# krullgit/3D-Object-Detection-for-autonomous-navigation

Measured on AMD Instinct MI355X. Metric: frames/sec (whole node) + p50 per-frame ms, 16k-pt pillars, higher is better.
Workload: dtype f32 (GEMMs on the 16-bit matrix pipe as split operands -- two float16 pieces per value, 3 products, fp32 accumulate: fp32-equivalent results, measured 1.5e-6 max from the fp32 oracle at this shape)

## Files before the change

### 3d-object-detection-for-autonomous-navigation_amd/csrc/voxelize.hip

```cpp
#include "pp_common.h"

#define VT 1024
#define VWAVES 16
#define VL_PPT 16
#define VL_CAP (VT * VL_PPT)

__device__ __forceinline__ unsigned long long lanemask_lt() {
    unsigned lane = threadIdx.x & 63u;
    return (lane == 0) ? 0ull : (~0ull >> (64u - lane));
}

__global__ __launch_bounds__(256) void k_cell_first(const float* __restrict__ pts,
                                                    const int* __restrict__ offsets, int F, VoxGeom g,
                                                    int* __restrict__ cell, int* __restrict__ first,
                                                    int* __restrict__ cellmap, const PpFeed* __restrict__ feed,
                                                    float* __restrict__ pts_dst, int* __restrict__ offsets_dst,
                                                    unsigned long long* __restrict__ occbits, int occ_n) {
    const int b = blockIdx.y;
    if (feed != nullptr) {
        offsets = feed->offsets;
        pts = feed->src;
    }
    if (cellmap != nullptr) {
        int* cm = cellmap + (size_t)b * g.ncell;
        if ((g.ncell & 3) == 0) {
            const int4 m1 = make_int4(-1, -1, -1, -1);
            for (int e = blockIdx.x * 256 + threadIdx.x; e < (g.ncell >> 2); e += gridDim.x * 256) reinterpret_cast<int4*>(cm)[e] = m1;
        } else {
            for (int e = blockIdx.x * 256 + threadIdx.x; e < g.ncell; e += gridDim.x * 256) cm[e] = -1;
        }
    }
    if (occbits != nullptr)
        for (int e = blockIdx.x * 256 + threadIdx.x; e < occ_n; e += gridDim.x * 256) occbits[(size_t)b * occ_n + e] = 0ull;
    const int n0 = offsets[b];
    const int n1 = offsets[b + 1];
    const int n = n1 - n0;
    if (feed != nullptr && blockIdx.x == 0 && threadIdx.x == 0) {
        offsets_dst[b] = n0;
        if (b == (int)gridDim.y - 1) offsets_dst[b + 1] = n1;
    }
    const int i = blockIdx.x * 256 + threadIdx.x;
    if (i >= n) return;
    const float* ps_ = pts + (size_t)(n0 + i) * F;
    float p[3] = {ps_[0], ps_[1], ps_[2]};
    if (feed != nullptr) {
        float* q = pts_dst + (size_t)(n0 + i) * F;
        q[0] = p[0]; q[1] = p[1]; q[2] = p[2];
        for (int j = 3; j < F; ++j) q[j] = ps_[j];
    }
    int c3[3];
    bool ok = true;
#pragma unroll
    for (int j = 0; j < 3; ++j) {
        double c = floor(((double)p[j] - g.lo[j]) / g.vs[j]);
        if (!(c >= 0.0 && c < (double)g.grid[j])) ok = false;
        c3[j] = ok ? (int)c : 0;
    }
    int lin = -1;
    if (ok) {
        lin = (c3[2] * g.grid[1] + c3[1]) * g.grid[0] + c3[0];
        if (first != nullptr) atomicMin(&first[(size_t)b * g.ncell + lin], i);
    }
    cell[n0 + i] = lin;
}

__device__ __forceinline__ int block_excl_scan(int v, int* s_tmp, int& total) {
    const int lane = threadIdx.x & 63, wave = threadIdx.x >> 6;
    const int x = wave_inclusive_scan(v);
    if (lane == 63) s_tmp[wave] = x;
    __syncthreads();
    int woff = 0, tot = 0;
#pragma unroll
    for (int w = 0; w < VWAVES; ++w) {
        int t = s_tmp[w];
        if (w < wave) woff += t;
        tot += t;
    }
    __syncthreads();
    total = tot;
    return woff + x - v;
}

int voxel_sort_passes(int max_voxels) {
    int bits = 1;
    while ((1 << bits) < max_voxels) ++bits;
    return (bits + 7) / 8;
}

template <int BITS, int PPT>
__global__ __launch_bounds__(VT) void k_voxel_frame(
    const int* __restrict__ offsets, const int* __restrict__ cell, const int* __restrict__ first,
    int* __restrict__ cellmap, unsigned* keyA, unsigned* idxA, unsigned* keyB, unsigned* idxB,
    int* __restrict__ pillar_start, int* __restrict__ pillar_cell, int* __restrict__ npillars,
    int* __restrict__ nvalid_out, int ncell, int max_voxels, int npass, int bits_rt) {
    const int bits = (BITS > 0) ? BITS : bits_rt;
    __shared__ int s_tot[VWAVES];
    __shared__ int s_carry;
    __shared__ int s_break;
    __shared__ int s_tmp[VWAVES];
    __shared__ int s_hist[256 * VWAVES];
    constexpr int CAP = VT * PPT;
    constexpr bool TABLES = (PPT == 16);
    __shared__ unsigned s_sort[2 * VL_CAP];

    const int b = blockIdx.x;
    const int tid = threadIdx.x, lane = tid & 63, wave = tid >> 6;
    const int n0 = offsets[b];
    const int n = offsets[b + 1] - n0;
    const int* fcell = cell + n0;
    const int* ffirst = (first != nullptr) ? first + (size_t)b * ncell : nullptr;
    int* fmap = cellmap + (size_t)b * ncell;
    unsigned* kA = keyA + n0;
    unsigned* vA = idxA + n0;
    unsigned* kB = keyB + n0;
    unsigned* vB = idxB + n0;
    const unsigned long long lt = lanemask_lt();

    if (tid == 0) { s_carry = 0; s_break = 0x7fffffff; }
    __syncthreads();

    int ib = 1;
    while ((1 << ib) < n) ++ib;
    if (n <= CAP && npass * bits + ib <= 32 && (first != nullptr || (TABLES && ncell <= VL_CAP))) {
        const int ppt = (n + VT - 1) / VT;
        const int i0 = tid * ppt;
        int c[PPT];
        if (ppt == PPT && ((n0 | n) & 3) == 0 && i0 + PPT <= n) {
#pragma unroll
            for (int k = 0; k < PPT; k += 4) {
                const int4 v = *reinterpret_cast<const int4*>(fcell + i0 + k);
                c[k] = v.x; c[k + 1] = v.y; c[k + 2] = v.z; c[k + 3] = v.w;
            }
        } else {
#pragma unroll
            for (int k = 0; k < PPT; ++k) c[k] = (k < ppt && i0 + k < n) ? fcell[i0 + k] : -1;
        }
        int f[PPT];
        if (first != nullptr) {
#pragma unroll
            for (int k = 0; k < PPT; ++k) f[k] = (c[k] >= 0) ? ffirst[c[k]] : -1;
        } else {
            int* s_first = reinterpret_cast<int*>(s_sort) + VL_CAP;
            for (int e = tid; e < ncell; e += VT) s_first[e] = 0x7fffffff;
            __syncthreads();
#pragma unroll
            for (int k = 0; k < PPT; ++k) if (c[k] >= 0) atomicMin(&s_first[c[k]], i0 + k);
            __syncthreads();
#pragma unroll
            for (int k = 0; k < PPT; ++k) f[k] = (c[k] >= 0) ? s_first[c[k]] : -1;
            __syncthreads();
        }
        int* const s_map = reinterpret_cast<int*>(s_sort) + VL_CAP;
        unsigned flags = 0;
#pragma unroll
        for (int k = 0; k < PPT; ++k) if (c[k] >= 0 && f[k] == i0 + k) flags |= 1u << k;
        int totp;
        const int basep = block_excl_scan(__popc(flags), s_tmp, totp);
        {
            int r = 0;
#pragma unroll
            for (int k = 0; k < PPT; ++k)
                if ((flags >> k) & 1u) {
                    const int pid = basep + r++;
                    if (pid < max_voxels) {
                        fmap[c[k]] = pid;
                        if (first == nullptr) s_map[c[k]] = pid;
                        pillar_cell[(size_t)b * max_voxels + pid] = c[k];
                    } else if (pid == max_voxels) {
                        s_break = i0 + k;
                    }
                }
        }
        __syncthreads();
        const int P = min(totp, max_voxels);
        const int ibreak = s_break;
        unsigned vmask = 0;
#pragma unroll
        for (int k = 0; k < PPT; ++k) if (c[k] >= 0 && i0 + k < ibreak) vmask |= 1u << k;
        int key[PPT];
#pragma unroll
        for (int k = 0; k < PPT; ++k) key[k] = ((vmask >> k) & 1u) ? (first == nullptr ? s_map[c[k]] : fmap[c[k]]) : 0;
        int nv;
        const int basev = block_excl_scan(__popc(vmask), s_tmp, nv);
        {
            int r = 0;
#pragma unroll
            for (int k = 0; k < PPT; ++k)
                if ((vmask >> k) & 1u) s_sort[basev + r++] = ((unsigned)key[k] << ib) | (unsigned)(i0 + k);
        }
        __syncthreads();
        unsigned* const sk = s_sort;
        unsigned* const dk = s_sort;
        const int NB = 1 << bits;
        const unsigned dmask = (unsigned)NB - 1u;
        const int chunk = ((nv + VWAVES * 64 - 1) / (VWAVES * 64)) * 64;
        const int wbeg = min(wave * chunk, nv), wend = min(wbeg + chunk, nv);
        for (int pass = 0; pass < npass; ++pass) {
            const int shift = ib + pass * bits;
            for (int e = tid; e < NB * VWAVES; e += VT) s_hist[e] = 0;
            unsigned ev[PPT];
#pragma unroll
            for (int t = 0; t < PPT; ++t) {
                const int j = wbeg + t * 64 + lane;
                ev[t] = (j < wend) ? sk[j] : 0u;
            }
            __syncthreads();
            int rank[PPT], rbase[PPT];
            const unsigned lt_lo = (unsigned)lt, lt_hi = (unsigned)(lt >> 32);
#pragma unroll
            for (int t = 0; t < PPT; ++t) {
                rank[t] = 0;
                rbase[t] = 0;
                if (wbeg + t * 64 < wend) {
                    const bool act = wbeg + t * 64 + lane < wend;
                    const unsigned d = (ev[t] >> shift) & dmask;
                    const unsigned long long am = __builtin_amdgcn_ballot_w64(act);
                    unsigned plo = (unsigned)am, phi = (unsigned)(am >> 32);
                    if (BITS > 0) {
#pragma unroll
                        for (int bit = 0; bit < BITS; ++bit) {
                            const unsigned m = (unsigned)__builtin_amdgcn_sbfe((int)d, bit, 1);
                            const unsigned long long bb = __builtin_amdgcn_ballot_w64(__builtin_amdgcn_ubfe(d, bit, 1) != 0u);
                            plo &= ~((unsigned)bb ^ m);
                            phi &= ~((unsigned)(bb >> 32) ^ m);
                        }
                    } else {
                        for (int bit = 0; bit < bits; ++bit) {
                            const unsigned m = (unsigned)__builtin_amdgcn_sbfe((int)d, bit, 1);
                            const unsigned long long bb = __builtin_amdgcn_ballot_w64(__builtin_amdgcn_ubfe(d, bit, 1) != 0u);
                            plo &= ~((unsigned)bb ^ m);
                            phi &= ~((unsigned)(bb >> 32) ^ m);
                        }
                    }
                    if (act) {
                        int* hp = &s_hist[wave * NB + d];
                        rbase[t] = __hip_atomic_load(hp, __ATOMIC_RELAXED, __HIP_MEMORY_SCOPE_WORKGROUP);
                        const unsigned blo = plo & lt_lo, bhi = phi & lt_hi;
                        rank[t] = __popc(blo) + __popc(bhi);
                        if ((blo | bhi) == 0u)
                            __hip_atomic_fetch_add(hp, __popc(plo) + __popc(phi), __ATOMIC_RELAXED, __HIP_MEMORY_SCOPE_WORKGROUP);
                    }
                }
            }
#pragma unroll
            for (int t = 0; t < PPT; ++t) rank[t] += rbase[t];
            __syncthreads();
            {
                const int E = NB * VWAVES;
                const int per = (E + VT - 1) / VT;
                const int e0 = tid * per;
                int local = 0;
                for (int q = 0; q < per; ++q)
                    if (e0 + q < E) local += s_hist[((e0 + q) % VWAVES) * NB + (e0 + q) / VWAVES];
                int total;
                int run = block_excl_scan(local, s_tmp, total);
                for (int q = 0; q < per; ++q)
                    if (e0 + q < E) {
                        int* hp = &s_hist[((e0 + q) % VWAVES) * NB + (e0 + q) / VWAVES];
                        const int t = *hp;
                        *hp = run;
                        run += t;
                    }
            }
            __syncthreads();
#pragma unroll
            for (int t = 0; t < PPT; ++t) {
                if (wbeg + t * 64 + lane < wend) {
                    const unsigned d = (ev[t] >> shift) & dmask;
                    dk[s_hist[wave * NB + d] + rank[t]] = ev[t];
                }
            }
            __syncthreads();
        }
        int* ps = pillar_start + (size_t)b * (max_voxels + 1);
        const unsigned imask = (1u << ib) - 1u;
        unsigned* fin = ((npass & 1) ? idxB : idxA) + n0;
#pragma unroll
        for (int t = 0; t < PPT; ++t) {
            const int j = tid + t * VT;
            if (j < nv) {
                const unsigned v = sk[j];
                fin[j] = v & imask;
                const unsigned k = v >> ib;
                if (j == 0 || (sk[j - 1] >> ib) != k) ps[k] = j;
            }
        }
        if (tid == 0) {
            ps[P] = nv;
            npillars[b] = P;
            nvalid_out[b] = nv;
        }
        return;
    }

    for (int base = 0; base < n; base += VT) {
        const int i = base + tid;
        const int c = (i < n) ? fcell[i] : -1;
        const bool flag = (c >= 0) && (ffirst[c] == i);
        const unsigned long long bal = __ballot(flag);
        if (lane == 0) s_tot[wave] = __popcll(bal);
        __syncthreads();
        int woff = 0, tile_tot = 0;
#pragma unroll
        for (int w = 0; w < VWAVES; ++w) {
            int t = s_tot[w];
            if (w < wave) woff += t;
            tile_tot += t;
        }
        const int pid = s_carry + woff + __popcll(bal & lt);
        if (flag) {
            if (pid < max_voxels) {
                fmap[c] = pid;
                pillar_cell[(size_t)b * max_voxels + pid] = c;
            } else if (pid == max_voxels) {
                s_break = i;
            }
        }
        __syncthreads();
        if (tid == 0) s_carry += tile_tot;
    }
    __syncthreads();
    const int P = min(s_carry, max_voxels);
    const int ibreak = s_break;
    __syncthreads();

    if (tid == 0) s_carry = 0;
    __syncthreads();
    for (int base = 0; base < n; base += VT) {
        const int i = base + tid;
        const int c = (i < n) ? fcell[i] : -1;
        const bool valid = (c >= 0) && (i < ibreak);
        const unsigned long long bal = __ballot(valid);
        if (lane == 0) s_tot[wave] = __popcll(bal);
        __syncthreads();
        int woff = 0, tile_tot = 0;
#pragma unroll
        for (int w = 0; w < VWAVES; ++w) {
            int t = s_tot[w];
            if (w < wave) woff += t;
            tile_tot += t;
        }
        if (valid) {
            const int pos = s_carry + woff + __popcll(bal & lt);
            kA[pos] = (unsigned)fmap[c];
            vA[pos] = (unsigned)i;
        }
        __syncthreads();
        if (tid == 0) s_carry += tile_tot;
    }
    __syncthreads();
    const int nv = s_carry;
    __syncthreads();

    unsigned* sk = kA; unsigned* sv = vA; unsigned* dk = kB; unsigned* dv = vB;
    const int NB = 1 << bits;
    const unsigned dmask = (unsigned)NB - 1u;
    const int chunk = ((nv + VWAVES * 64 - 1) / (VWAVES * 64)) * 64;
    const int wbeg = min(wave * chunk, nv);
    const int wend = min(wbeg + chunk, nv);
    volatile int* vhist = s_hist;
    for (int pass = 0; pass < npass; ++pass) {
        const int shift = pass * bits;
        for (int e = tid; e < NB * VWAVES; e += VT) s_hist[e] = 0;
        __syncthreads();
        for (int t0 = wbeg; t0 < wend; t0 += 64) {
            const int j = t0 + lane;
            if (j < wend) atomicAdd(&s_hist[wave * NB + ((sk[j] >> shift) & dmask)], 1);
        }
        __syncthreads();
        {
            const int E = NB * VWAVES;
            const int per = (E + VT - 1) / VT;
            const int e0 = tid * per;
            int local = 0;
            for (int q = 0; q < per; ++q)
                if (e0 + q < E) local += s_hist[((e0 + q) % VWAVES) * NB + (e0 + q) / VWAVES];
            int total;
            int run = block_excl_scan(local, s_tmp, total);
            for (int q = 0; q < per; ++q)
                if (e0 + q < E) {
                    int* hp = &s_hist[((e0 + q) % VWAVES) * NB + (e0 + q) / VWAVES];
                    const int t = *hp;
                    *hp = run;
                    run += t;
                }
        }
        __syncthreads();
        for (int t0 = wbeg; t0 < wend; t0 += 64) {
            const int j = t0 + lane;
            const bool act = j < wend;
            const unsigned k = act ? sk[j] : 0u;
            const unsigned v = act ? sv[j] : 0u;
            const unsigned d = (k >> shift) & dmask;
            unsigned long long peers = __ballot(act);
            for (int bit = 0; bit < bits; ++bit) {
                const bool one = (d >> bit) & 1u;
                const unsigned long long bb = __ballot(act && one);
                peers &= one ? bb : ~bb;
            }
            if (act) {
                const int basep = vhist[wave * NB + d];
                const int pos = basep + __popcll(peers & lt);
                dk[pos] = k;
                dv[pos] = v;
                if (lane == 63 - __clzll(peers)) vhist[wave * NB + d] = basep + __popcll(peers);
            }
        }
        __syncthreads();
        unsigned* t;
        t = sk; sk = dk; dk = t;
        t = sv; sv = dv; dv = t;
    }

    int* ps = pillar_start + (size_t)b * (max_voxels + 1);
    for (int j = tid; j < nv; j += VT) {
        const unsigned k = sk[j];
        if (j == 0 || sk[j - 1] != k) ps[k] = j;
    }
    if (tid == 0) {
        ps[P] = nv;
        npillars[b] = P;
        nvalid_out[b] = nv;
    }
}

__global__ __launch_bounds__(256) void k_sort_points(const float* __restrict__ pts, const int* __restrict__ offsets,
                                                     const unsigned* __restrict__ idx, const int* __restrict__ nvalid,
                                                     int F, float* __restrict__ pts_sorted, int batch, int nchunk) {
    const int xcd = blockIdx.x & 7, r = blockIdx.x >> 3;
    const int chunk = r % nchunk, b = (r / nchunk) * 8 + xcd;
    if (b >= batch) return;
    const int j = chunk * 256 + threadIdx.x;
    if (j >= nvalid[b]) return;
    const int n0 = offsets[b];
    const unsigned src = idx[n0 + j];
    const float* fp = pts + (size_t)(n0 + src) * F;
    float* fs = pts_sorted + (size_t)(n0 + j) * F;
    if (F == 4) {
        *reinterpret_cast<float4*>(fs) = *reinterpret_cast<const float4*>(fp);
    } else {
        const float x = fp[0], y = fp[1], z = fp[2];
        fs[0] = x; fs[1] = y; fs[2] = z;
    }
}

__global__ __launch_bounds__(64) void k_voxel_expand(const float* __restrict__ pts_sorted,
                                                     const int* __restrict__ offsets,
                                                     const unsigned* __restrict__ sorted_idx,
                                                     const int* __restrict__ pillar_start,
                                                     const int* __restrict__ pillar_cell,
                                                     const int* __restrict__ npillars, int frame, int F, int T,
                                                     int max_voxels, int ny, int nx, float* __restrict__ voxels,
                                                     int* __restrict__ coors, int* __restrict__ num_points) {
    const int p = blockIdx.x;
    if (p >= npillars[frame]) return;
    const int n0 = offsets[frame];
    const int* ps = pillar_start + (size_t)frame * (max_voxels + 1);
    const int start = ps[p];
    const int cnt = min(ps[p + 1] - start, T);
    (void)sorted_idx;
    for (int e = threadIdx.x; e < T * F; e += 64) {
        const int s = e / F, f = e - s * F;
        float v = 0.f;
        if (s < cnt) v = pts_sorted[(size_t)(n0 + start + s) * F + f];
        voxels[((size_t)p * T) * F + e] = v;
    }
    if (threadIdx.x == 0) {
        const int c = pillar_cell[(size_t)frame * max_voxels + p];
        const int x = c % nx, y = (c / nx) % ny, z = c / (nx * ny);
        coors[p * 3 + 0] = z;
        coors[p * 3 + 1] = y;
        coors[p * 3 + 2] = x;
        num_points[p] = cnt;
    }
}

__global__ __launch_bounds__(256) void k_build_cellmap(const int* __restrict__ coors4, int64_t P, int ncell,
                                                       int ny, int nx, int* __restrict__ cellmap) {
    const int64_t p = (int64_t)blockIdx.x * 256 + threadIdx.x;
    if (p >= P) return;
    const int b = coors4[p * 4 + 0], z = coors4[p * 4 + 1], y = coors4[p * 4 + 2], x = coors4[p * 4 + 3];
    cellmap[(size_t)b * ncell + ((size_t)z * ny + y) * nx + x] = (int)p;
}

bool voxel_first_in_lds(int max_n, int ncell, int max_voxels) {
    int kb = 1, ib = 1;
    while ((1 << kb) < max_voxels) ++kb;
    while ((1 << ib) < max_n) ++ib;
    const int npass = (kb + 7) / 8;
    const int bits = (kb + npass - 1) / npass;
    return max_n <= VL_CAP && ncell <= VL_CAP && npass * bits + ib <= 32;
}

void launch_cell_first(const float* pts, const int* offsets, int batch, int max_n, int F, const VoxGeom& g,
                       int* cell, int* first, int* cellmap, const PpFeed* feed, float* pts_dst, int* offsets_dst,
                       hipStream_t s, unsigned long long* occbits, int occ_n) {
    if (batch <= 0) return;
    dim3 grid(max_n > 0 ? (max_n + 255) / 256 : 1, batch);
    PP_LAUNCH("k_cell_first", k_cell_first, grid, dim3(256), 0, s, pts, offsets, F, g, cell, first, cellmap, feed, pts_dst,
              offsets_dst, occbits, occ_n);
}

void launch_voxel_frame(const int* offsets, const int* cell, const int* first, int* cellmap, unsigned* keyA,
                        unsigned* idxA, unsigned* keyB, unsigned* idxB, int* pillar_start, int* pillar_cell,
                        int* npillars, int* nvalid, int batch, int max_n, int ncell, int max_voxels, hipStream_t s) {
    if (batch <= 0) return;
    int kb = 1;
    while ((1 << kb) < max_voxels) ++kb;
    const int npass = (kb + 7) / 8;
    const int bits = (kb + npass - 1) / npass;
    const bool big = max_n > VL_CAP;
#define VOX_LAUNCH(B_, P_)                                                                                            \
    PP_LAUNCH("k_voxel_frame", (k_voxel_frame<B_, P_>), dim3(batch), dim3(VT), 0, s, offsets, cell, first, cellmap, keyA, \
              idxA, keyB, idxB, pillar_start, pillar_cell, npillars, nvalid, ncell, max_voxels, npass, bits)
    if (bits == 7) {
        if (big) VOX_LAUNCH(7, 32); else VOX_LAUNCH(7, 16);
    } else {
        if (big) VOX_LAUNCH(0, 32); else VOX_LAUNCH(0, 16);
    }
#undef VOX_LAUNCH
}

__global__ __launch_bounds__(256) void k_fill_first(int* __restrict__ first, int v, long long n) {
    for (long long i = (long long)blockIdx.x * blockDim.x + threadIdx.x; i < n; i += (long long)gridDim.x * blockDim.x)
        first[i] = v;
}

void launch_fill_first(int* first, int v, long long n, hipStream_t s) {
    if (n <= 0) return;
    const long long blocks = std::min<long long>((n + 255) / 256, 8192);
    PP_LAUNCH("k_fill_first", k_fill_first, dim3((unsigned)blocks), dim3(256), 0, s, first, v, n);
}

void launch_sort_points(const float* pts, const int* offsets, const unsigned* sorted_idx, const int* nvalid, int batch,
                        int max_n, int F, float* pts_sorted, hipStream_t s) {
    if (batch <= 0 || max_n <= 0) return;
    const int nchunk = (max_n + 255) / 256;
    PP_LAUNCH("k_sort_points", k_sort_points, dim3(8 * nchunk * ((batch + 7) / 8)), dim3(256), 0, s, pts, offsets,
              sorted_idx, nvalid, F, pts_sorted, batch, nchunk);
}

void launch_voxel_expand(const float* pts, const int* offsets, const unsigned* sorted_idx, const int* pillar_start,
                         const int* pillar_cell, const int* npillars, int frame, int F, int T, int max_voxels,
                         int ny, int nx, float* voxels, int* coors, int* num_points, hipStream_t s) {
    PP_LAUNCH("k_voxel_expand", k_voxel_expand, dim3(max_voxels), dim3(64), 0, s, pts, offsets, sorted_idx, pillar_start,
                       pillar_cell, npillars, frame, F, T, max_voxels, ny, nx, voxels, coors, num_points);
}

void launch_build_cellmap(const int* coors4, int64_t P, int ncell, int ny, int nx, int* cellmap, hipStream_t s) {
    if (P <= 0) return;
    PP_LAUNCH("k_build_cellmap", k_build_cellmap, dim3((unsigned)((P + 255) / 256)), dim3(256), 0, s, coors4, P, ncell, ny,
                       nx, cellmap);
}
```

Before: 93850.

## Size voxel-frame LDS dynamically and shrink cell map to 16-bit entries

```diff
diff --git a/3d-object-detection-for-autonomous-navigation_amd/csrc/voxelize.hip b/3d-object-detection-for-autonomous-navigation_amd/csrc/voxelize.hip
--- a/3d-object-detection-for-autonomous-navigation_amd/csrc/voxelize.hip
+++ b/3d-object-detection-for-autonomous-navigation_amd/csrc/voxelize.hip
@@ -1,9 +1,12 @@
 #include "pp_common.h"
 
-#define VT 1024
-#define VWAVES 16
-#define VL_PPT 16
-#define VL_CAP (VT * VL_PPT)
+#include <algorithm>
+#include <mutex>
+#include <set>
+#include <utility>
+
+#define VL_CAP 16384
+#define VOX_THREADS 1024
 
 __device__ __forceinline__ unsigned long long lanemask_lt() {
     unsigned lane = threadIdx.x & 63u;
@@ -64,6 +67,7 @@
     cell[n0 + i] = lin;
 }
 
+template <int NW>
 __device__ __forceinline__ int block_excl_scan(int v, int* s_tmp, int& total) {
     const int lane = threadIdx.x & 63, wave = threadIdx.x >> 6;
     const int x = wave_inclusive_scan(v);
@@ -71,7 +75,7 @@
     __syncthreads();
     int woff = 0, tot = 0;
 #pragma unroll
-    for (int w = 0; w < VWAVES; ++w) {
+    for (int w = 0; w < NW; ++w) {
         int t = s_tmp[w];
         if (w < wave) woff += t;
         tot += t;
@@ -87,21 +91,22 @@
     return (bits + 7) / 8;
 }
 
-template <int BITS, int PPT>
-__global__ __launch_bounds__(VT) void k_voxel_frame(
+template <int BITS, int PPT, int NT>
+__global__ __launch_bounds__(NT) void k_voxel_frame(
     const int* __restrict__ offsets, const int* __restrict__ cell, const int* __restrict__ first,
     int* __restrict__ cellmap, unsigned* keyA, unsigned* idxA, unsigned* keyB, unsigned* idxB,
     int* __restrict__ pillar_start, int* __restrict__ pillar_cell, int* __restrict__ npillars,
-    int* __restrict__ nvalid_out, int ncell, int max_voxels, int npass, int bits_rt) {
+    int* __restrict__ nvalid_out, int ncell, int max_voxels, int npass, int bits_rt, int sort_cap) {
+    constexpr int VT = NT, VWAVES = NT / 64;
     const int bits = (BITS > 0) ? BITS : bits_rt;
     __shared__ int s_tot[VWAVES];
     __shared__ int s_carry;
     __shared__ int s_break;
     __shared__ int s_tmp[VWAVES];
-    __shared__ int s_hist[256 * VWAVES];
+    extern __shared__ int s_dyn[];
+    int* const s_hist = s_dyn;
+    unsigned* const s_sort = reinterpret_cast<unsigned*>(s_dyn) + (VWAVES << bits);
     constexpr int CAP = VT * PPT;
-    constexpr bool TABLES = (PPT == 16);
-    __shared__ unsigned s_sort[2 * VL_CAP];
 
     const int b = blockIdx.x;
     const int tid = threadIdx.x, lane = tid & 63, wave = tid >> 6;
@@ -121,7 +126,7 @@
 
     int ib = 1;
     while ((1 << ib) < n) ++ib;
-    if (n <= CAP && npass * bits + ib <= 32 && (first != nullptr || (TABLES && ncell <= VL_CAP))) {
+    if (n <= CAP && n <= sort_cap && npass * bits + ib <= 32) {
         const int ppt = (n + VT - 1) / VT;
         const int i0 = tid * ppt;
         int c[PPT];
@@ -140,7 +145,7 @@
 #pragma unroll
             for (int k = 0; k < PPT; ++k) f[k] = (c[k] >= 0) ? ffirst[c[k]] : -1;
         } else {
-            int* s_first = reinterpret_cast<int*>(s_sort) + VL_CAP;
+            int* s_first = reinterpret_cast<int*>(s_sort);
             for (int e = tid; e < ncell; e += VT) s_first[e] = 0x7fffffff;
             __syncthreads();
 #pragma unroll
@@ -150,12 +155,12 @@
             for (int k = 0; k < PPT; ++k) f[k] = (c[k] >= 0) ? s_first[c[k]] : -1;
             __syncthreads();
         }
-        int* const s_map = reinterpret_cast<int*>(s_sort) + VL_CAP;
+        unsigned short* const s_map = reinterpret_cast<unsigned short*>(s_sort + sort_cap);
         unsigned flags = 0;
 #pragma unroll
         for (int k = 0; k < PPT; ++k) if (c[k] >= 0 && f[k] == i0 + k) flags |= 1u << k;
         int totp;
-        const int basep = block_excl_scan(__popc(flags), s_tmp, totp);
+        const int basep = block_excl_scan<VWAVES>(__popc(flags), s_tmp, totp);
         {
             int r = 0;
 #pragma unroll
@@ -164,7 +169,7 @@
                     const int pid = basep + r++;
                     if (pid < max_voxels) {
                         fmap[c[k]] = pid;
-                        if (first == nullptr) s_map[c[k]] = pid;
+                        if (first == nullptr) s_map[c[k]] = (unsigned short)pid;
                         pillar_cell[(size_t)b * max_voxels + pid] = c[k];
                     } else if (pid == max_voxels) {
                         s_break = i0 + k;
@@ -179,9 +184,9 @@
         for (int k = 0; k < PPT; ++k) if (c[k] >= 0 && i0 + k < ibreak) vmask |= 1u << k;
         int key[PPT];
 #pragma unroll
-        for (int k = 0; k < PPT; ++k) key[k] = ((vmask >> k) & 1u) ? (first == nullptr ? s_map[c[k]] : fmap[c[k]]) : 0;
+        for (int k = 0; k < PPT; ++k) key[k] = ((vmask >> k) & 1u) ? (first == nullptr ? (int)s_map[c[k]] : fmap[c[k]]) : 0;
         int nv;
-        const int basev = block_excl_scan(__popc(vmask), s_tmp, nv);
+        const int basev = block_excl_scan<VWAVES>(__popc(vmask), s_tmp, nv);
         {
             int r = 0;
 #pragma unroll
@@ -253,7 +258,7 @@
                 for (int q = 0; q < per; ++q)
                     if (e0 + q < E) local += s_hist[((e0 + q) % VWAVES) * NB + (e0 + q) / VWAVES];
                 int total;
-                int run = block_excl_scan(local, s_tmp, total);
+                int run = block_excl_scan<VWAVES>(local, s_tmp, total);
                 for (int q = 0; q < per; ++q)
                     if (e0 + q < E) {
                         int* hp = &s_hist[((e0 + q) % VWAVES) * NB + (e0 + q) / VWAVES];
@@ -376,7 +381,7 @@
             for (int q = 0; q < per; ++q)
                 if (e0 + q < E) local += s_hist[((e0 + q) % VWAVES) * NB + (e0 + q) / VWAVES];
             int total;
-            int run = block_excl_scan(local, s_tmp, total);
+            int run = block_excl_scan<VWAVES>(local, s_tmp, total);
             for (int q = 0; q < per; ++q)
                 if (e0 + q < E) {
                     int* hp = &s_hist[((e0 + q) % VWAVES) * NB + (e0 + q) / VWAVES];
@@ -501,6 +506,20 @@
               offsets_dst, occbits, occ_n);
 }
 
+static void voxel_frame_allow_lds(const void* kernel) {
+    static std::mutex mu;
+    static std::set<std::pair<const void*, int>> done;
+    int dev = 0, lds = 0;
+    if (hipGetDevice(&dev) != hipSuccess) return;
+    std::lock_guard<std::mutex> lock(mu);
+    if (done.count({kernel, dev})) return;
+    hipFuncAttributes fa;
+    if (hipFuncGetAttributes(&fa, kernel) == hipSuccess &&
+        hipDeviceGetAttribute(&lds, hipDeviceAttributeMaxSharedMemoryPerBlock, dev) == hipSuccess &&
+        hipFuncSetAttribute(kernel, hipFuncAttributeMaxDynamicSharedMemorySize, lds - (int)fa.sharedSizeBytes) == hipSuccess)
+        done.insert({kernel, dev});
+}
+
 void launch_voxel_frame(const int* offsets, const int* cell, const int* first, int* cellmap, unsigned* keyA,
                         unsigned* idxA, unsigned* keyB, unsigned* idxB, int* pillar_start, int* pillar_cell,
                         int* npillars, int* nvalid, int batch, int max_n, int ncell, int max_voxels, hipStream_t s) {
@@ -509,10 +528,17 @@
     while ((1 << kb) < max_voxels) ++kb;
     const int npass = (kb + 7) / 8;
     const int bits = (kb + npass - 1) / npass;
+    const int tables = (first == nullptr) ? ((ncell + 63) / 64) * 64 : 0;
+    const int sort_cap = std::max(((std::min(std::max(max_n, 1), 2 * VL_CAP) + 63) / 64) * 64, tables);
+    const size_t lds_bytes = (size_t)sort_cap * 4 + (size_t)tables * 2 + (size_t)((VOX_THREADS / 64) << bits) * 4;
     const bool big = max_n > VL_CAP;
 #define VOX_LAUNCH(B_, P_)                                                                                            \
-    PP_LAUNCH("k_voxel_frame", (k_voxel_frame<B_, P_>), dim3(batch), dim3(VT), 0, s, offsets, cell, first, cellmap, keyA, \
-              idxA, keyB, idxB, pillar_start, pillar_cell, npillars, nvalid, ncell, max_voxels, npass, bits)
+    do {                                                                                                              \
+        voxel_frame_allow_lds(reinterpret_cast<const void*>(&k_voxel_frame<B_, P_, VOX_THREADS>));                    \
+        PP_LAUNCH("k_voxel_frame", (k_voxel_frame<B_, P_, VOX_THREADS>), dim3(batch), dim3(VOX_THREADS), lds_bytes, s, \
+                  offsets, cell, first, cellmap, keyA, idxA, keyB, idxB, pillar_start, pillar_cell, npillars, nvalid, \
+                  ncell, max_voxels, npass, bits, sort_cap);                                                          \
+    } while (0)
     if (bits == 7) {
         if (big) VOX_LAUNCH(7, 32); else VOX_LAUNCH(7, 16);
     } else {
```

Measured after the change: 93310, median of 2. About the same (-0.6%).
